# matteociccozzi/LayoutDiT

Measured on AMD Instinct MI355X. Metric: images/sec ViT-B/16 224px bs=64 fwd, higher is better.
Workload: dtype f32; 1 GPU; ViT-base/16 224x224 bs=64 f32 forward, taps [4, 6, 8, 12] (BASELINE.json configs[1]); images_per_gpu=64, global_batch=64, parallelism=dp1: batch-sharded replicas, no data-path collective, weights=synthetic seed 0, images=synthetic doc-like pages, seed 1234, rank0_placement=128 CPUs: NUMA node 0 of GPU 0000:23:00.0

## Files before the change

layoutdit_amd/csrc/api.hip:

```cpp
#include "api_internal.h"

namespace ldit {

char *err_buf()
{
    static thread_local char buf[512] = {0};
    return buf;
}

int fail(int code, const char *fmt, ...)
{
    va_list ap;
    va_start(ap, fmt);
    vsnprintf(err_buf(), 512, fmt, ap);
    va_end(ap);
    return code;
}

int ensure_dynamic_lds(const void *kern, int bytes, std::atomic<unsigned long long> &done)
{
    int dev = 0;
    LDIT_HIP_CHECK(hipGetDevice(&dev));
    const unsigned long long bit = dev >= 0 && dev < 64 ? 1ull << dev : 0ull;
    if (bit && (done.load(std::memory_order_relaxed) & bit)) return LDIT_OK;
    LDIT_HIP_CHECK(hipFuncSetAttribute(kern, hipFuncAttributeMaxDynamicSharedMemorySize, bytes));
    if (bit) done.fetch_or(bit, std::memory_order_relaxed);
    return LDIT_OK;
}

int compute_units()
{
    static std::atomic<int> cached[64];
    int dev = 0;
    if (hipGetDevice(&dev) != hipSuccess) return 256;
    const bool slot = dev >= 0 && dev < 64;
    if (slot) {
        const int c = cached[dev].load(std::memory_order_relaxed);
        if (c > 0) return c;
    }
    int n = 0;
    if (hipDeviceGetAttribute(&n, hipDeviceAttributeMultiprocessorCount, dev) != hipSuccess || n <= 0) n = 256;
    if (slot) cached[dev].store(n, std::memory_order_relaxed);
    return n;
}

namespace {
DiagSwitches read_switches()
{
    DiagSwitches d;
    auto digit = [](const char *name, int lo, int hi) {
        const char *e = getenv(name);
        return (e && e[0] >= '0' + lo && e[0] <= '0' + hi && e[1] == 0) ? e[0] - '0' : -1;
    };
    auto is = [](const char *name, char c) { const char *e = getenv(name); return e && e[0] == c; };
    d.gemm_tile = digit("LDIT_GEMM_TILE", 0, 7);
    if (const char *e = getenv("LDIT_GEMM_THIN_TILES")) d.thin_tiles = atol(e);
    d.panel_r16_vec = is("LDIT_PANEL_R16", 'v');
    d.panel_persist = is("LDIT_GEMM_PERSIST", '1');
    d.bf16_tile = digit("LDIT_GEMM_BF16_TILE", 2, 7);
    d.bf16_tile_env = getenv("LDIT_GEMM_BF16_TILE") != nullptr;
    d.bf16_tr_tile = digit("LDIT_GEMM_BF16_TR_TILE", 0, 9);
    d.bf16_tail_launch = is("LDIT_GEMM_BF16_TAIL_LAUNCH", '1');
    d.fp8_tile = digit("LDIT_GEMM_FP8_TILE", 0, 6);
    d.fp8_k16 = is("LDIT_GEMM_FP8_K16", '1');
    d.fp8_noskinny = is("LDIT_GEMM_FP8_NOSKINNY", '1');
    d.direct_epi = is("LDIT_GEMM_DIRECT_EPILOGUE", '1');
    d.attn_bf16_kt4 = is("LDIT_ATTN_BF16_KT", '4');
    d.seg_order = digit("LDIT_GEMM_SEG_ORDER", 0, 1);
    if (const char *e = getenv("LDIT_PLANES_TAIL_WAVES")) d.planes_tail_waves = atol(e);
    d.attn_bf16_nw = digit("LDIT_ATTN_BF16_NW", 4, 8);
    return d;
}
DiagSwitches &switches()
{
    static DiagSwitches d = read_switches();
    return d;
}
}

const DiagSwitches &diag() { return switches(); }
void reload_diag() { switches() = read_switches(); }

int embed(const Geo &g, const float *x, const float *pw, const float *pb, const float *cls, const float *pos, float *out,
          int batch, int img_h, int img_w, hipStream_t stream, Probe &probe)
{
    GemmArgs a{};
    a.A = x; a.W = pw; a.Y = out; a.Y2 = nullptr; a.bias = pb; a.pos = pos;
    a.M = batch * g.P; a.N = g.C; a.K = g.Kp;
    a.lda = g.in_ch * img_h * img_w;
    a.ldy = g.C;
    a.img_h = img_h; a.img_w = img_w; a.gw = g.gw; a.patches = g.P; a.patch = g.p; a.tokens = g.T;
    LDIT_RUN(probe, LDIT_K_GEMM, launch_gemm(a, EPI_EMBED, A_PATCH, stream));
    LDIT_RUN(probe, LDIT_K_OTHER, launch_cls_rows(cls, pos, out, batch, g.T, g.C, stream));
    return LDIT_OK;
}

int embed_bf16(const Geo &g, const float *x, const ImgSrc *imgs, int planes, void *patches, const void *w16, const float *pb,
               const float *cls, const float *pos, float *out, int batch, int img_h, int img_w, hipStream_t stream, Probe &probe)
{
    if (imgs)
        LDIT_RUN(probe, LDIT_K_OTHER, launch_patches_rows_images(imgs->images, imgs->half_in, imgs->heights, imgs->widths, batch, g.in_ch,
                                                                imgs->mean, imgs->std, img_h, img_w, g.p, patches, stream, planes));
    else
        LDIT_RUN(probe, LDIT_K_OTHER, launch_patches_rows(x, patches, batch, g.in_ch, img_h, img_w, g.p, stream, planes));
    GemmExtra xe = split_segments(planes);
    xe.pos = pos; xe.patches = g.P;
    LDIT_RUN(probe, LDIT_K_GEMM, launch_gemm_bf16_ex(patches, planes * g.Kp, w16, pb, out, g.C, batch * g.P, g.C, g.Kp, EPI_EMBED, nullptr,
                                                    nullptr, nullptr, xe, stream));
    LDIT_RUN(probe, LDIT_K_OTHER, launch_cls_rows(cls, pos, out, batch, g.T, g.C, stream));
    return LDIT_OK;
}

int layernorm(Build b, const float *X, const float *gamma, const float *beta, const Operand &Y, void *Yd, int64_t rows, int C, float eps, hipStream_t stream)
{
    switch (b.dtype) {
        case LDIT_F32: return launch_layernorm(X, gamma, beta, static_cast<float *>(Y.p), rows, C, eps, stream);
        case LDIT_BF16: return launch_layernorm_bf16out(X, gamma, beta, Y.p, rows, C, eps, stream);
        case LDIT_FP8: return launch_layernorm_fp8out(X, gamma, beta, Y.p, rows, C, eps, static_cast<const float *>(Y.s), stream);
        case LDIT_MXFP8:
            return b.train ? launch_layernorm_mxout_train(X, gamma, beta, Y.p, Y.s, Yd, rows, C, eps, stream)
                           : launch_layernorm_mxout(X, gamma, beta, Y.p, Y.s, rows, C, eps, stream);
        case LDIT_F32X3: case LDIT_F32X6: return launch_layernorm_splitout(X, gamma, beta, Y.p, rows, C, eps, Y.planes, stream);
        default: return fail(LDIT_EUNSUPPORTED, "layernorm: no kernel for dtype %d", b.dtype);
    }
}

int linear(Build b, const Operand &A, const void *W, const void *Ws, const float *bias, const Operand &Y, int M, int N, int K, int epi,
           const float *lam, const float *R, float *Y2, const Side &t, hipStream_t stream, float ab_scale, float out_inv_scale)
{
    switch (b.dtype) {
        case LDIT_F32: {
            GemmArgs a{};
            a.A = static_cast<const float *>(A.p); a.W = static_cast<const float *>(W); a.Y = static_cast<float *>(Y.p); a.Y2 = Y2;
            a.bias = bias; a.lam = lam; a.R = R;
            a.M = M; a.N = N; a.K = K; a.lda = A.ld; a.ldy = Y.ld;
            return launch_gemm(a, epi, A_ROWMAJOR, stream);
        }
        case LDIT_BF16: case LDIT_F32X3: case LDIT_F32X6: {
            GemmExtra x = split_segments(A.planes);
            x.Ypre = t.Ypre; x.rowscale = t.rowscale;
            if (Y.planes) { x.nsplit_out = Y.planes; epi = epi == EPI_BIAS_GELU ? EPI_GELU_SPLIT : EPI_BIAS_SPLIT; }
            return launch_gemm_bf16_ex(A.p, A.ld, W, bias, Y.p, Y.ld, M, N, K, epi, lam, R, Y2, x, stream);
        }
        case LDIT_FP8:
            return launch_gemm_fp8(A.p, A.ld, W, bias, Y.p, Y.ld, M, N, K, epi, lam, R, Y2, ab_scale, out_inv_scale,
                                   static_cast<const float *>(A.s), static_cast<const float *>(Ws), static_cast<const float *>(Y.s), stream);
        case LDIT_MXFP8:
            if (b.train && epi != EPI_BIAS)
                return launch_gemm_mxfp8_train(A.p, A.ld, A.s, W, Ws, bias, Y.p, Y.ld, Y.s, M, N, K, epi, lam, R, Y2, t.Ypre, t.rowscale, t.Yd, stream);
            return launch_gemm_mxfp8(A.p, A.ld, A.s, W, Ws, bias, Y.p, Y.ld, Y.s, M, N, K, epi, lam, R, Y2, stream);
        default: return fail(LDIT_EUNSUPPORTED, "linear: no kernel for dtype %d", b.dtype);
    }
}

int attention(Build b, const void *Q, const void *K, const void *V, int ldq, int ldk, int ldv, const Operand &O, int B, int N, int H, int D,
              float scale, hipStream_t stream, float *lse, void *Ob, void *Od, int plane_in)
{
    switch (b.dtype) {
        case LDIT_F32:
            return launch_attention(static_cast<const float *>(Q), static_cast<const float *>(K), static_cast<const float *>(V),
                                    static_cast<float *>(O.p), B, N, H, D, ldq, ldk, ldv, O.ld, scale, stream);
        case LDIT_BF16:
            return b.train ? launch_attention_bf16_lse(Q, K, V, O.p, lse, B, N, H, D, ldq, ldk, ldv, O.ld, scale, stream)
                           : launch_attention_bf16(Q, K, V, O.p, B, N, H, D, ldq, ldk, ldv, O.ld, scale, stream);
        case LDIT_FP8:
            return launch_attention_bf16_fp8out(Q, K, V, O.p, B, N, H, D, ldq, ldk, ldv, O.ld, scale, static_cast<const float *>(O.s), stream);
        case LDIT_MXFP8:
            return b.train ? launch_attention_bf16_mxout_train(Q, K, V, O.p, O.s, lse, Ob, Od, B, N, H, D, ldq, ldk, ldv, O.ld, scale, stream)
                           : launch_attention_bf16_mxout(Q, K, V, O.p, O.s, B, N, H, D, ldq, ldk, ldv, O.ld, scale, stream);
        case LDIT_F32X3: case LDIT_F32X6:
            return (O.planes == 2 ? launch_attention_planes2 : launch_attention_planes3)(Q, K, V, O.p, B, N, H, D, ldq, plane_in, O.ld, stream);
        default: return fail(LDIT_EUNSUPPORTED, "attention: no kernel for dtype %d", b.dtype);
    }
}

int run_layer(Build b, const Geo &g, int batch, float eps, const Layer &d, hipStream_t stream, Probe &probe)
{
    const int M = batch * g.T, C = g.C, F = g.F;
    const char *q = static_cast<const char *>(d.qkv.p), *k = q + d.qk_bytes, *v = k + d.qk_bytes;
    const Operand mid = operand(d.h_mid, nullptr, C), out = operand(d.h_out, nullptr, C);
    const PackedLayer &pv = *d.v, &pw = *d.w;
    LDIT_RUN(probe, LDIT_K_LAYERNORM, layernorm(b, d.h_in, d.vec(pv.ln1_w), d.vec(pv.ln1_b), d.y1, d.y1d, M, C, eps, stream));
    LDIT_RUN(probe, LDIT_K_GEMM, linear(b, d.y1, d.mat(pw.wqkv), d.W + pw.sw_qkv, d.bqkv, d.qkv, M, 3 * C, C, EPI_BIAS, nullptr, nullptr, nullptr, Side{}, stream));
    LDIT_RUN(probe, LDIT_K_ATTENTION, attention(b, q, k, v, d.qkv.ld, d.qkv.ld, d.qkv.ld, d.o, batch, g.T, g.H, g.D, d.scale, stream, d.lse, d.ob, d.od,
                                                d.qkv.planes ? d.qkv.ld / d.qkv.planes : 0));
    LDIT_RUN(probe, LDIT_K_GEMM, linear(b, d.o, d.mat(pw.wo), d.W + pw.sw_o, d.vec(pv.bo), mid, M, C, C, EPI_SCALE_RESID, d.vec(pv.lam1), d.h_in, nullptr, d.s_o, stream));
    LDIT_RUN(probe, LDIT_K_LAYERNORM, layernorm(b, d.h_mid, d.vec(pv.ln2_w), d.vec(pv.ln2_b), d.y2, d.y2d, M, C, eps, stream));
    LDIT_RUN(probe, LDIT_K_GEMM, linear(b, d.y2, d.mat(pw.w1), d.W + pw.sw_1, d.vec(pv.b1), d.hid, M, F, C, EPI_BIAS_GELU, nullptr, nullptr, nullptr, d.s_fc1, stream));
    LDIT_RUN(probe, LDIT_K_GEMM, linear(b, d.hid, d.mat(pw.w2), d.W + pw.sw_2, d.vec(pv.b2), out, M, C, F, EPI_SCALE_RESID, d.vec(pv.lam2), d.h_mid, d.tap, d.s_fc2, stream));
    return LDIT_OK;
}

namespace {

Geo embed_geo(int64_t in_ch, int64_t img_h, int64_t img_w, int64_t p, int64_t C)
{
    Geo g{};
    g.C = (int)C; g.p = (int)p; g.in_ch = (int)in_ch; g.gh = (int)(img_h / p); g.gw = (int)(img_w / p);
    g.P = g.gh * g.gw; g.T = g.P + 1; g.Kp = (int)(in_ch * p * p);
    return g;
}

int embed_bf16_entry(const char *name, const void *x, const ImgSrc *imgs, const void *patch_w_bf16, const void *patch_b, const void *cls,
                     const void *pos, void *out, void *scratch, int64_t B, int64_t in_ch, int64_t img_h, int64_t img_w, int64_t p, int64_t C,
                     ldit_stream stream)
{
    if (B <= 0 || (imgs && B > 65535) || in_ch <= 0 || img_h <= 0 || img_w <= 0 || p <= 0 || C <= 0) return fail(LDIT_EINVAL, "%s: empty problem", name);
    if (img_h % p || img_w % p)
        return fail(LDIT_EINVAL, "%s: %s %lldx%lld is not a multiple of patch %lld", name, imgs ? "target" : "image", (long long)img_h, (long long)img_w, (long long)p);
    if ((imgs ? !imgs->images || !imgs->heights || !imgs->widths : !x) || !patch_w_bf16 || !patch_b || !cls || !pos || !out || !scratch)
        return fail(LDIT_EINVAL, "%s: null operand", name);
    if (imgs && !(imgs->std > 0.0f)) return fail(LDIT_EINVAL, "%s: std must be positive", name);
    if (!aligned16(out) || !aligned16(pos) || !aligned16(scratch) || !aligned16(patch_w_bf16) || (C & 3))
        return fail(LDIT_EINVAL, "%s: out / pos / scratch / patch_w must be 16-byte aligned, C a multiple of 4", name);
    const int64_t P = (img_h / p) * (img_w / p), Kp = in_ch * p * p;
    if (Kp % 64) return fail(LDIT_EUNSUPPORTED, "%s: in_ch*p*p = %lld must be a multiple of 64", name, (long long)Kp);
    if (B * in_ch * img_h * img_w >= (1ll << 31) || B * (P + 1) * C >= (1ll << 31) || B * P * Kp >= (1ll << 31))
        return fail(LDIT_EUNSUPPORTED, "%s: operand exceeds 2^31 elements", name);
    Probe probe;
    return embed_bf16(embed_geo(in_ch, img_h, img_w, p, C), static_cast<const float *>(x), imgs, 1, scratch, patch_w_bf16,
                      static_cast<const float *>(patch_b), static_cast<const float *>(cls), static_cast<const float *>(pos), static_cast<float *>(out),
                      (int)B, (int)img_h, (int)img_w, static_cast<hipStream_t>(stream), probe);
}
// ... 516 lines not shown
```

layoutdit_amd/csrc/attention_f32.hip:

```cpp
#include "ldit_common.h"

#ifdef LDIT_GEMM_STAMPS
__device__ unsigned long long *g_attn32_stamps = nullptr;
#define A32_STAMP(var) const unsigned long long var = __builtin_amdgcn_s_memtime()
#else
#define A32_STAMP(var)
#endif

namespace ldit {

namespace {

constexpr int KSTR = 68;
constexpr int VSTR = 64;

template <int KT, int NW>
__global__ void __launch_bounds__(NW * 64, NW == 4 ? 2 : NW / 4) attention_f32(const float *__restrict__ Q, const float *__restrict__ K,
                                                     const float *__restrict__ V, float *__restrict__ O, int N, int H,
                                                     int ldq, int ldk, int ldv, int ldo, float scale, int nqg)
{
    constexpr int KROWS = KT * 32;
    extern __shared__ __attribute__((aligned(16))) char smem[];
    float *Ks = reinterpret_cast<float *>(smem);
    float *Vs = Ks + KROWS * KSTR;

    const int tid = threadIdx.x, lane = tid & 63;
    const int wave = __builtin_amdgcn_readfirstlane(tid >> 6);
    const int li = lane & 31, lh = lane >> 5;
    const int bid = blockIdx.x;
    const int qg = bid % nqg, bh = bid / nqg, head = bh % H, b = bh / H;
    const int qt = qg * NW + wave;
    const bool active = qt * 32 < N;
    const size_t tok0 = (size_t)b * N;
#ifdef LDIT_GEMM_STAMPS
    unsigned long long ph[4] = {0, 0, 0, 0};
#endif
    A32_STAMP(t_begin);

    float q[32];
    {
        int qrow = qt * 32 + li;
        qrow = qrow < N ? qrow : N - 1;
        const f32x4 *qp = reinterpret_cast<const f32x4 *>(Q + (tok0 + qrow) * ldq + head * 64 + 32 * lh);
#pragma unroll
        for (int u = 0; u < 8; ++u) {
            const f32x4 t = qp[u];
            q[4 * u + 0] = t[0]; q[4 * u + 1] = t[1]; q[4 * u + 2] = t[2]; q[4 * u + 3] = t[3];
        }
    }

    f32x16 o[2];
#pragma unroll
    for (int e = 0; e < 16; ++e) { o[0][e] = 0.0f; o[1][e] = 0.0f; }
    float m_run = -INFINITY, l_run = 0.0f;

    for (int c0 = 0; c0 < N; c0 += KROWS) {
        const int nkeys = (N - c0) < KROWS ? (N - c0) : KROWS;
        const int ktiles = (nkeys + 31) >> 5;
        A32_STAMP(t0);
        if (c0) __syncthreads();
        {
            constexpr int PER = (32 * 16) / (NW * 64) > 0 ? (32 * 16) / (NW * 64) : 1;
            static_assert((32 * 16) % (NW * 64) == 0, "a key tile must split evenly over the threads");
            constexpr int BATCH = 4;
#pragma unroll
            for (int e = 0; e < PER; ++e)
#pragma unroll
                for (int k0 = 0; k0 < KT; k0 += BATCH) {
                    f32x4 kv[BATCH], vv[BATCH];
#pragma unroll
                    for (int i = 0; i < BATCH; ++i) {
                        const int kt = k0 + i, u = kt * 512 + e * NW * 64 + tid, row = u >> 4, c4 = (u & 15) * 4;
                        kv[i] = f32x4{0.f, 0.f, 0.f, 0.f};
                        vv[i] = f32x4{0.f, 0.f, 0.f, 0.f};
                        if (kt < KT && kt < ktiles && row < nkeys) {
                            kv[i] = *reinterpret_cast<const f32x4 *>(K + (tok0 + c0 + row) * ldk + head * 64 + c4);
                            vv[i] = *reinterpret_cast<const f32x4 *>(V + (tok0 + c0 + row) * ldv + head * 64 + c4);
                        }
                    }
#pragma unroll
                    for (int i = 0; i < BATCH; ++i) {
                        const int kt = k0 + i, u = kt * 512 + e * NW * 64 + tid, row = u >> 4, c4 = (u & 15) * 4;
                        if (kt < KT && kt < ktiles) {
                            *reinterpret_cast<f32x4 *>(Ks + row * KSTR + c4) = kv[i];
                            *reinterpret_cast<f32x4 *>(Vs + row * VSTR + c4) = vv[i];
                        }
                    }
                }
        }
        __syncthreads();
        if (!active) continue;
        A32_STAMP(t1);

        f32x16 s[KT];
#pragma unroll
        for (int kt = 0; kt < KT; ++kt) {
#pragma unroll
            for (int e = 0; e < 16; ++e) s[kt][e] = 0.0f;
            if (kt < ktiles) {
                const float *kr = Ks + (kt * 32 + li) * KSTR + 32 * lh;
#pragma unroll
                for (int u = 0; u < 8; ++u) {
                    const f32x4 kf = *reinterpret_cast<const f32x4 *>(kr + 4 * u);
#pragma unroll
                    for (int e = 0; e < 4; ++e)
                        s[kt] = __builtin_amdgcn_mfma_f32_32x32x2f32(kf[e], q[4 * u + e], s[kt], 0, 0, 0);
                }
            }
        }
#ifdef LDIT_GEMM_STAMPS
        asm volatile("s_nop 0" ::"v"(s[0][0]), "v"(s[KT - 1][0]));
#endif
        A32_STAMP(t2);
        float mx = -INFINITY;
#pragma unroll
        for (int kt = 0; kt < KT; ++kt) {
            if (kt < ktiles) {
                const bool partial = (kt + 1) * 32 > nkeys;
#pragma unroll
                for (int r = 0; r < 16; ++r) {
                    float v = s[kt][r] * scale;
                    if (partial && (kt * 32 + 8 * (r >> 2) + 4 * lh + (r & 3)) >= nkeys) v = -INFINITY;
                    s[kt][r] = v;
                    mx = fmaxf(mx, v);
                }
            }
        }
        mx = fmaxf(mx, __shfl_xor(mx, 32, 64));
        const float m_new = fmaxf(m_run, mx);
        const float alpha = __expf(m_run - m_new);
        m_run = m_new;
        float lsum = 0.0f;
#pragma unroll
        for (int kt = 0; kt < KT; ++kt) {
            if (kt < ktiles) {
#pragma unroll
                for (int r = 0; r < 16; ++r) {
                    const float pv = __expf(s[kt][r] - m_new);
                    s[kt][r] = pv;
                    lsum += pv;
                }
            }
        }
        l_run = l_run * alpha + lsum;
        if (c0) {
#pragma unroll
            for (int e = 0; e < 16; ++e) { o[0][e] *= alpha; o[1][e] *= alpha; }
        }
        A32_STAMP(t3);
#pragma unroll
        for (int kt = 0; kt < KT; ++kt) {
            if (kt < ktiles) {
                const int left = nkeys - kt * 32;
#pragma unroll
                for (int r = 0; r < 16; ++r) {
                    if (8 * (r >> 2) + (r & 3) >= left) continue;
                    const float *vr = Vs + (kt * 32 + 8 * (r >> 2) + 4 * lh + (r & 3)) * VSTR + li;
                    o[0] = __builtin_amdgcn_mfma_f32_32x32x2f32(vr[0], s[kt][r], o[0], 0, 0, 0);
                    o[1] = __builtin_amdgcn_mfma_f32_32x32x2f32(vr[32], s[kt][r], o[1], 0, 0, 0);
                }
            }
        }
#ifdef LDIT_GEMM_STAMPS
        asm volatile("s_nop 0" ::"v"(o[0][0]), "v"(o[1][0]));
        ph[0] += t1 - t0 + (c0 ? 0 : t0 - t_begin); ph[1] += t2 - t1; ph[2] += t3 - t2; ph[3] += __builtin_amdgcn_s_memtime() - t3;
#endif
    }

    if (!active) return;
#ifdef LDIT_GEMM_STAMPS
    if (g_attn32_stamps && wave == 0 && lane == 0) {
        unsigned long long *d = g_attn32_stamps + (size_t)blockIdx.x * 6;
        d[0] = ph[0]; d[1] = ph[1]; d[2] = ph[2]; d[3] = ph[3]; d[5] = __builtin_amdgcn_s_memtime() - t_begin;
    }
#endif
    const float l = l_run + __shfl_xor(l_run, 32, 64);
    const float inv = 1.0f / l;
    const int qrow = qt * 32 + li;
    if (qrow < N) {
        float *op = O + (tok0 + qrow) * ldo + head * 64 + 4 * lh;
#pragma unroll
        for (int dt = 0; dt < 2; ++dt)
#pragma unroll
            for (int g = 0; g < 4; ++g) {
                f32x4 t = {o[dt][4 * g + 0] * inv, o[dt][4 * g + 1] * inv, o[dt][4 * g + 2] * inv, o[dt][4 * g + 3] * inv};
                *reinterpret_cast<f32x4 *>(op + dt * 32 + 8 * g) = t;
            }
    }
}

}

int launch_attention(const float *Q, const float *K, const float *V, float *O, int B, int N, int H, int D, int ldq,
                     int ldk, int ldv, int ldo, float scale, hipStream_t stream)
{
    if (B <= 0 || N <= 0 || H <= 0) return fail(LDIT_EINVAL, "attention: empty problem");
    if (D != 64) return fail(LDIT_EUNSUPPORTED, "attention: head_dim=%d, only 64 is implemented", D);
    if (!Q || !K || !V || !O) return fail(LDIT_EINVAL, "attention: null operand");
    if ((ldq | ldk | ldv | ldo) & 3) return fail(LDIT_EINVAL, "attention: row strides must be multiples of 4 floats");
    if (!aligned16(Q) || !aligned16(K) || !aligned16(V) || !aligned16(O)) return fail(LDIT_EINVAL, "attention: operands must be 16-byte aligned");
    constexpr int KT = 7;
    constexpr int lds = KT * 32 * (KSTR + VSTR) * 4;
    const int nqt = (N + 31) / 32;
    auto go = [&](auto kern, int nw, std::atomic<unsigned long long> &attr_done) -> int {
        if (int rc = ensure_dynamic_lds(reinterpret_cast<const void *>(kern), lds, attr_done)) return rc;
        const int nqg = (nqt + nw - 1) / nw;
        hipLaunchKernelGGL(kern, dim3((unsigned)(B * H * nqg)), dim3(nw * 64), lds, stream, Q, K, V, O, N, H, ldq, ldk, ldv, ldo,
                           scale, nqg);
        LDIT_HIP_CHECK(hipGetLastError());
        return LDIT_OK;
    };
    static std::atomic<unsigned long long> set8{0}, set4{0};
    const long wgs8 = (long)B * H * ((nqt + 7) / 8);
    if (wgs8 <= 128 && nqt > 4) { if (int rc = go(attention_f32<KT, 4>, 4, set4)) return rc; }
    else if (int rc = go(attention_f32<KT, 8>, 8, set8)) return rc;
    LDIT_HIP_CHECK(hipGetLastError());
    return LDIT_OK;
}

}

#ifdef LDIT_GEMM_STAMPS
extern "C" int ldit_dbg_set_attn32_stamps(void *buf)
{
    unsigned long long *p = static_cast<unsigned long long *>(buf);
    return hipMemcpyToSymbol(HIP_SYMBOL(g_attn32_stamps), &p, sizeof(p)) == hipSuccess ? 0 : -3;
}
#endif
```

layoutdit_amd/csrc/ldit_common.h:

```cpp
#pragma once
#include <hip/hip_runtime.h>

#include <atomic>
#include <cstdarg>
#include <cstdint>
#include <cstdio>

#include "ldit.h"

namespace ldit {

typedef float f32x2 __attribute__((ext_vector_type(2)));
typedef float f32x4 __attribute__((ext_vector_type(4)));
typedef float f32x16 __attribute__((ext_vector_type(16)));

char *err_buf();
int fail(int code, const char *fmt, ...);

#define LDIT_HIP_CHECK(expr)                                                                              \
    do {                                                                                                  \
        hipError_t e__ = (expr);                                                                          \
        if (e__ != hipSuccess) return ::ldit::fail(LDIT_EHIP, "%s: %s", #expr, hipGetErrorString(e__));   \
    } while (0)

static inline bool aligned16(const void *p) { return (reinterpret_cast<uintptr_t>(p) & 15u) == 0; }

int ensure_dynamic_lds(const void *kern, int bytes, std::atomic<unsigned long long> &done);
#define LDIT_DYN_LDS(kern, bytes)                                                                               \
    do {                                                                                                        \
        static std::atomic<unsigned long long> done__{0};                                                       \
        if (int rc__ = ::ldit::ensure_dynamic_lds(reinterpret_cast<const void *>(kern), (bytes), done__)) return rc__; \
    } while (0)

int compute_units();

struct DiagSwitches {
    int gemm_tile = -1;
    long thin_tiles = 192;
    bool panel_r16_vec = false;
    bool panel_persist = false;
    int bf16_tile = -1;
    bool bf16_tile_env = false;
    int bf16_tr_tile = -1;
    bool bf16_tail_launch = false;
    int fp8_tile = -1;
    bool fp8_k16 = false, fp8_noskinny = false;
    bool direct_epi = false;
    bool attn_bf16_kt4 = false;
    int attn_bf16_nw = -1;
    long planes_tail_waves = 700;
    int seg_order = -1;
};
const DiagSwitches &diag();
void reload_diag();

__device__ __forceinline__ float erf_fast(float a)
{
    const float t = fabsf(a), s = a * a;
    float r = fmaf(-1.72853470e-5f, t, 3.83197126e-4f);
    const float u = fmaf(-3.88396438e-3f, t, 2.42546219e-2f);
    r = fmaf(r, s, u);
    r = fmaf(r, t, -1.06777877e-1f);
    r = fmaf(r, t, -6.34846687e-1f);
    r = fmaf(r, t, -1.28717512e-1f);
    r = fmaf(r, t, -t);
    const float big = copysignf(1.0f - __expf(r), a);
    float q = -5.96761703e-4f;
    q = fmaf(q, s, 4.99119423e-3f);
    q = fmaf(q, s, -2.67681349e-2f);
    q = fmaf(q, s, 1.12819925e-1f);
    q = fmaf(q, s, -3.76125336e-1f);
    q = fmaf(q, s, 1.28379166e-1f);
    const float small = fmaf(q, a, a);
    return t > 0.927734375f ? big : small;
}

__device__ __forceinline__ float gelu_erf(float v) { return 0.5f * v * (1.0f + erf_fast(v * 0.70710678118654752440f)); }

__device__ __forceinline__ float gelu_lp(float v)
{
    const float w = v * __builtin_fmaf(v * v, -0.10294324f, -2.30220819f);
    return v * __builtin_amdgcn_rcpf(1.0f + __builtin_amdgcn_exp2f(w));
}

__device__ __forceinline__ void gelu_and_grad_lp(float v, float &gelu, float &grad)
{
    const float v2 = v * v;
    const float w = v * __builtin_fmaf(v2, -0.10294324f, -2.30220819f);
    const float s = __builtin_amdgcn_rcpf(1.0f + __builtin_amdgcn_exp2f(w));
    const float vs = v * s;
    gelu = vs;
    grad = __builtin_fmaf(vs - vs * s, __builtin_fmaf(v2, 0.21406445f, 1.59576912f), s);
}

__device__ __forceinline__ unsigned pack_fp8x4(float a, float b, float c, float d)
{
    const float lim = 448.0f;
    a = fminf(fmaxf(a, -lim), lim); b = fminf(fmaxf(b, -lim), lim);
    c = fminf(fmaxf(c, -lim), lim); d = fminf(fmaxf(d, -lim), lim);
    int w = 0;
    w = __builtin_amdgcn_cvt_pk_fp8_f32(a, b, w, false);
    w = __builtin_amdgcn_cvt_pk_fp8_f32(c, d, w, true);
    return (unsigned)w;
}

__device__ __forceinline__ unsigned umax32(unsigned a, unsigned b) { return a > b ? a : b; }

__device__ __forceinline__ unsigned mx_scale_byte(unsigned amax)
{
    if (amax >= 0x7f800000u) return 0xFFu;
    if (amax == 0u) return 0u;
    int e = (int)(amax >> 23) - 135 + ((amax & 0x7fffffu) > 0x600000u ? 1 : 0);
    e = e < -127 ? -127 : (e > 127 ? 127 : e);
    return (unsigned)(e + 127);
}

__device__ __forceinline__ float mx_inv_scale(unsigned b) { return b >= 254u ? 1.0f : __uint_as_float((254u - b) << 23); }

__device__ __forceinline__ float mx_scale_value(unsigned b)
{
    return b == 0u ? __uint_as_float(0x00400000u) : (b == 255u ? __uint_as_float(0x7fc00000u) : __uint_as_float(b << 23));
}

typedef __bf16 mx_bf16x4 __attribute__((ext_vector_type(4)));

__device__ __forceinline__ mx_bf16x4 mx_dequant_bf16x4(unsigned pk, unsigned b)
{
    const float s = mx_scale_value(b);
    return mx_bf16x4{(__bf16)(__builtin_amdgcn_cvt_f32_fp8((int)pk, 0) * s), (__bf16)(__builtin_amdgcn_cvt_f32_fp8((int)pk, 1) * s),
                     (__bf16)(__builtin_amdgcn_cvt_f32_fp8((int)pk, 2) * s), (__bf16)(__builtin_amdgcn_cvt_f32_fp8((int)pk, 3) * s)};
}

enum AMode { A_ROWMAJOR = 0, A_PATCH = 1,
             A_CONV3 = 2 };
enum Epi { EPI_BIAS = 0, EPI_BIAS_GELU = 1, EPI_SCALE_RESID = 2, EPI_EMBED = 3,
           EPI_F32 = 4,
           EPI_GELU_BWD = 5,
           EPI_GELU_SPLIT = 6,
           EPI_BIAS_SPLIT = 7 };

struct GemmExtra {
    void *Ypre = nullptr;
    const float *rowscale = nullptr;
    const void *aux = nullptr;
    int ldaux = 0;
    int splits = 1;
    const void *zeros = nullptr;
    const float *pos = nullptr;
    int patches = 0;
    int nseg = 0;
    unsigned seg_a = 0, seg_w = 0;
    int seg_inner = 0;
    int nsplit_out = 0;
    float *colsum = nullptr;
    int tail_rows = 0;
};

template <int S>
__device__ __forceinline__ void split_bf16_planes(float x, __bf16 (&p)[S])
{
#pragma unroll
    for (int s = 0; s < S; ++s) {
        p[s] = (__bf16)x;
        x -= (float)p[s];
    }
}

struct GemmArgs {
    const float *A;
    const float *W;
    float *Y;
    float *Y2;
    const float *bias;
    const float *lam;
    const float *R;
    const float *pos;
    int M, N, K;
    int lda, ldy;
    int img_h, img_w, gw, patches, patch, tokens;
    int conv_h, conv_w, conv_c;
    const float *zeros;
#ifdef LDIT_GEMM_STAMPS
    unsigned long long *stamps;
#endif
};

int launch_gemm(const GemmArgs &a, int epi, int amode, hipStream_t stream);
int launch_gemm_panel(const GemmArgs &a, int epi, int amode, hipStream_t stream, int height = 304);
int launch_gemm_thin(const GemmArgs &a, int epi, hipStream_t stream);
bool gemm_thin_prefers(int M, int N);

int launch_layernorm(const float *X, const float *g, const float *b, float *Y, int64_t rows, int C, float eps,
                     hipStream_t stream);
int launch_layernorm_bf16out(const float *X, const float *g, const float *b, void *Y, int64_t rows, int C, float eps,
                             hipStream_t stream);
int launch_attention_bf16(const void *Q, const void *K, const void *V, void *O, int B, int N, int H, int D, int ldq, int ldk,
                          int ldv, int ldo, float scale, hipStream_t stream);
int launch_attention(const float *Q, const float *K, const float *V, float *O, int B, int N, int H, int D, int ldq,
                     int ldk, int ldv, int ldo, float scale, hipStream_t stream);
int launch_cls_rows(const float *cls, const float *pos, float *out, int B, int tokens, int C, hipStream_t stream);
int launch_tap_to_map(const float *tap, float *out, int B, int Gh, int Gw, int C, float scale, hipStream_t stream);
int launch_tap_to_map_bwd(const float *dmap, float *dtap, int B, int Gh, int Gw, int C, float scale, hipStream_t stream);
// ... 105 lines not shown
```

layoutdit_amd/ops.py:

```python
from __future__ import annotations

import ctypes as C
from typing import Optional, Sequence

import torch

from . import _lib


def _device(*tensors) -> torch.device:
    dev = None
    for t in tensors:
        if t is None:
            continue
        if dev is None:
            dev = t.device
        elif t.device != dev:
            raise ValueError(f"tensor arguments live on different devices ({dev} and {t.device})")
    if dev is None or dev.type != "cuda":
        raise ValueError("expected tensors on the GPU (libldit_hip has no CPU path)")
    return dev


def _launch(dev: torch.device, fn, *args) -> None:
    with torch.cuda.device(dev):
        _lib.check(fn(*args, torch.cuda.current_stream(dev).cuda_stream))


def _req(t: torch.Tensor, name: str) -> torch.Tensor:
    if not isinstance(t, torch.Tensor) or not t.is_cuda:
        raise ValueError(f"{name}: expected a tensor on the GPU (libldit_hip has no CPU path)")
    if t.dtype != torch.float32:
        raise ValueError(f"{name}: expected float32, got {t.dtype}")
    if not t.is_contiguous():
        raise ValueError(f"{name}: expected a contiguous tensor")
    return t


def _ptr(t: Optional[torch.Tensor]):
    return None if t is None else t.data_ptr()


def linear(x: torch.Tensor, weight: torch.Tensor, bias: Optional[torch.Tensor] = None, epilogue: int = _lib.EPI_BIAS,
           lam: Optional[torch.Tensor] = None, residual: Optional[torch.Tensor] = None,
           out: Optional[torch.Tensor] = None, out2: Optional[torch.Tensor] = None) -> torch.Tensor:
    lib = _lib.load()
    x, weight = _req(x, "x"), _req(weight, "weight")
    M, K = x.shape
    N = weight.shape[0]
    if weight.shape[1] != K:
        raise ValueError(f"weight {tuple(weight.shape)} does not match x {tuple(x.shape)}")
    if out is None:
        out = torch.empty((M, N), device=x.device, dtype=torch.float32)
    for t, n in ((bias, "bias"), (lam, "lam"), (residual, "residual"), (out, "out"), (out2, "out2")):
        if t is not None:
            _req(t, n)
    _launch(_device(x, weight, bias, lam, residual, out, out2), lib.ldit_linear_f32, _ptr(x), K, _ptr(weight), _ptr(bias), _ptr(out), N, M, N, K, epilogue, _ptr(lam),
                                   _ptr(residual), _ptr(out2))
    return out


def layernorm(x: torch.Tensor, gamma: torch.Tensor, beta: torch.Tensor, eps: float = 1e-12) -> torch.Tensor:
    lib = _lib.load()
    x, gamma, beta = _req(x, "x"), _req(gamma, "gamma"), _req(beta, "beta")
    C = x.shape[-1]
    rows = x.numel() // C
    y = torch.empty_like(x)
    _launch(_device(x, gamma, beta), lib.ldit_layernorm_f32, _ptr(x), _ptr(gamma), _ptr(beta), _ptr(y), rows, C, eps)
    return y


def attention(q: torch.Tensor, k: torch.Tensor, v: torch.Tensor, heads: int, scale: Optional[float] = None) -> torch.Tensor:
    lib = _lib.load()
    for t, n in ((q, "q"), (k, "k"), (v, "v")):
        if not t.is_cuda or t.dtype != torch.float32 or t.stride(-1) != 1 or t.stride(0) != t.shape[1] * t.stride(1):
            raise ValueError(f"{n}: expected GPU float32 [B,N,H*D] with unit last stride and dense batch stride")
    B, N, HD = q.shape
    D = HD // heads
    o = torch.empty((B, N, HD), device=q.device, dtype=torch.float32)
    _launch(_device(q, k, v), lib.ldit_attention_f32, _ptr(q), _ptr(k), _ptr(v), _ptr(o), B, N, heads, D, q.stride(1), k.stride(1),
                                      v.stride(1), HD, float(D ** -0.5 if scale is None else scale))
    return o


def embed(x: torch.Tensor, patch_w: torch.Tensor, patch_b: torch.Tensor, cls: torch.Tensor, pos: torch.Tensor,
          patch: int) -> torch.Tensor:
    lib = _lib.load()
    x, patch_w, patch_b = _req(x, "x"), _req(patch_w, "patch_w"), _req(patch_b, "patch_b")
    cls, pos = _req(cls, "cls"), _req(pos, "pos")
    B, in_ch, H, W = x.shape
    Cc = patch_w.shape[0]
    T = (H // patch) * (W // patch) + 1
    out = torch.empty((B, T, Cc), device=x.device, dtype=torch.float32)
    _launch(_device(x, patch_w, patch_b, cls, pos), lib.ldit_embed_f32, _ptr(x), _ptr(patch_w), _ptr(patch_b), _ptr(cls), _ptr(pos), _ptr(out), B, in_ch, H, W,
                                  patch, Cc)
    return out


def embed_bf16(x: torch.Tensor, patch_w_bf16: torch.Tensor, patch_b: torch.Tensor, cls: torch.Tensor, pos: torch.Tensor,
               patch: int) -> torch.Tensor:
    lib = _lib.load()
    x, patch_b, cls, pos = _req(x, "x"), _req(patch_b, "patch_b"), _req(cls, "cls"), _req(pos, "pos")
    if patch_w_bf16.dtype != torch.bfloat16 or not patch_w_bf16.is_contiguous():
        raise ValueError("patch_w_bf16 must be a contiguous bfloat16 tensor")
    B, in_ch, H, W = x.shape
    Cc = patch_w_bf16.shape[0]
    P = (H // patch) * (W // patch)
    out = torch.empty((B, P + 1, Cc), device=x.device, dtype=torch.float32)
    scratch = torch.empty((B * P, in_ch * patch * patch), device=x.device, dtype=torch.bfloat16)
    _launch(_device(x, patch_w_bf16, patch_b, cls, pos), lib.ldit_embed_bf16, _ptr(x), _ptr(patch_w_bf16), _ptr(patch_b), _ptr(cls),
            _ptr(pos), _ptr(out), _ptr(scratch), B, in_ch, H, W, patch, Cc)
    return out


def tap_to_map(tap: torch.Tensor, gh: int, gw: int, scale: float) -> torch.Tensor:
    lib = _lib.load()
    tap = _req(tap, "tap")
    B, T, Cc = tap.shape
    if T != gh * gw + 1:
        raise ValueError(f"tap has {T} tokens, grid {gh}x{gw} needs {gh * gw + 1}")
    out = torch.empty((B, Cc, int(gh * scale), int(gw * scale)), device=tap.device, dtype=torch.float32)
    _launch(_device(tap), lib.ldit_tap_to_map_f32, _ptr(tap), _ptr(out), B, gh, gw, Cc, float(scale))
    return out


def _req16(t: torch.Tensor, name: str) -> torch.Tensor:
    if not isinstance(t, torch.Tensor) or not t.is_cuda or t.dtype != torch.float16 or not t.is_contiguous():
        raise ValueError(f"{name}: expected a contiguous float16 tensor on the GPU")
    return t


def widen_f16(x: torch.Tensor) -> torch.Tensor:
    lib = _lib.load()
    x = _req16(x, "x")
    out = torch.empty(x.shape, device=x.device, dtype=torch.float32)
    _launch(_device(x), lib.ldit_cast_f16_f32, _ptr(x), _ptr(out), x.numel())
    return out


def narrow_f16(x: torch.Tensor) -> torch.Tensor:
    lib = _lib.load()
    x = _req(x, "x")
    out = torch.empty(x.shape, device=x.device, dtype=torch.float16)
    _launch(_device(x), lib.ldit_cast_f32_f16, _ptr(x), _ptr(out), x.numel())
    return out


class _TapToMapFn(torch.autograd.Function):

    @staticmethod
    def forward(ctx, tap, gh, gw, scale):
        ctx.geom = (gh, gw, float(scale))
        return tap_to_map(tap.detach(), gh, gw, scale)

    @staticmethod
    def backward(ctx, dmap):
        gh, gw, scale = ctx.geom
        lib = _lib.load()
        dmap = _req(dmap.contiguous(), "dmap")
        B, Cc = dmap.shape[0], dmap.shape[1]
        dtap = torch.empty((B, gh * gw + 1, Cc), device=dmap.device, dtype=torch.float32)
        _launch(_device(dmap), lib.ldit_tap_to_map_bwd_f32, _ptr(dmap), _ptr(dtap), B, gh, gw, Cc, scale)
        return dtap, None, None, None


def tap_to_map_autograd(tap: torch.Tensor, gh: int, gw: int, scale: float) -> torch.Tensor:
    return _TapToMapFn.apply(tap, gh, gw, scale)


def preprocess(images: Sequence[torch.Tensor], size=224, mean: float = 0.5, std: float = 0.5) -> torch.Tensor:
    lib = _lib.load()
    imgs, ptrs, hs, ws, half, ch = image_list_args(images)
    B = len(imgs)
    out_h, out_w = (size, size) if isinstance(size, int) else (int(size[0]), int(size[1]))
    out = torch.empty((B, ch, out_h, out_w), device=imgs[0].device, dtype=torch.float32)
    if half:
        _launch(_device(*imgs), lib.ldit_preprocess_f16, ptrs, hs, ws, B, ch, mean, std, out_h, out_w, _ptr(out))
    else:
        _launch(_device(*imgs), lib.ldit_preprocess_f32, ptrs, hs, ws, B, ch, mean, std, out_h, out_w, _ptr(out))
    return out


def image_list_args(images: Sequence[torch.Tensor]):
    if len(images) == 0:
        raise ValueError("empty image list")
    half = images[0].dtype == torch.float16
    imgs = [(_req16 if half else _req)(t, f"images[{i}]") for i, t in enumerate(images)]
    ch = imgs[0].shape[0]
    if any(t.dim() != 3 or t.shape[0] != ch for t in imgs):
        raise ValueError("every image must be [C, h, w] with the same C")
    B = len(imgs)
    ptrs = (C.c_void_p * B)(*[t.data_ptr() for t in imgs])
    hs = (C.c_int32 * B)(*[t.shape[1] for t in imgs])
    ws = (C.c_int32 * B)(*[t.shape[2] for t in imgs])
    return imgs, ptrs, hs, ws, half, ch


def embed_bf16_images(images: Sequence[torch.Tensor], patch_w_bf16: torch.Tensor, patch_b: torch.Tensor, cls: torch.Tensor,
                      pos: torch.Tensor, patch: int, size=224, mean: float = 0.5, std: float = 0.5) -> torch.Tensor:
    lib = _lib.load()
    imgs, ptrs, hs, ws, half, ch = image_list_args(images)
    patch_b, cls, pos = _req(patch_b, "patch_b"), _req(cls, "cls"), _req(pos, "pos")
    if patch_w_bf16.dtype != torch.bfloat16 or not patch_w_bf16.is_contiguous():
        raise ValueError("patch_w_bf16 must be a contiguous bfloat16 tensor")
    out_h, out_w = (size, size) if isinstance(size, int) else (int(size[0]), int(size[1]))
    B, Cc = len(imgs), patch_w_bf16.shape[0]
    P = (out_h // patch) * (out_w // patch)
    dev = imgs[0].device
    out = torch.empty((B, P + 1, Cc), device=dev, dtype=torch.float32)
    scratch = torch.empty((B * P, ch * patch * patch), device=dev, dtype=torch.bfloat16)
    _launch(_device(*imgs, patch_w_bf16, patch_b, cls, pos), lib.ldit_embed_bf16_images, ptrs, hs, ws, int(half), mean, std,
            _ptr(patch_w_bf16), _ptr(patch_b), _ptr(cls), _ptr(pos), _ptr(out), _ptr(scratch), B, ch, out_h, out_w, patch, Cc)
    return out


def cast_bf16(x: torch.Tensor) -> torch.Tensor:
    lib = _lib.load()
    x = _req(x, "x")
    out = torch.empty(x.shape, device=x.device, dtype=torch.bfloat16)
    _launch(_device(x), lib.ldit_cast_f32_bf16, _ptr(x), _ptr(out), x.numel())
    return out


def linear_bf16(x: torch.Tensor, weight: torch.Tensor, bias: Optional[torch.Tensor] = None, epilogue: int = _lib.EPI_BIAS,
                lam: Optional[torch.Tensor] = None, residual: Optional[torch.Tensor] = None,
                out: Optional[torch.Tensor] = None, out2: Optional[torch.Tensor] = None) -> torch.Tensor:
    lib = _lib.load()
    for t, n in ((x, "x"), (weight, "weight")):
        if not t.is_cuda or t.dtype != torch.bfloat16 or not t.is_contiguous():
            raise ValueError(f"{n}: expected a contiguous bfloat16 GPU tensor")
    M, K = x.shape
    N = weight.shape[0]
# ... 839 lines not shown
```

Before: 3414 images/sec.

## Add persistent pipelined f32 attention kernel with direct-to-LDS K/V prefetch

Adds a persistent attention kernel, used when the whole key sequence fits in one LDS tile. Each block loops over (batch, head) pairs and prefetches the next head's K and Q with global_load_lds while the current head's PV product runs. It computes softmax in a single pass, since every key is resident, and XOR-swizzles the K rows in LDS instead of padding them. The old online-softmax kernel stays as the fallback, and the shared pieces are factored into helper functions. In exchange, the new path relies on inline assembly that manipulates m0, needs hand-placed waitcnt and barriers, and leaves one of the eight waves idle when the sequence has 197 tokens.

```diff
diff --git a/layoutdit_amd/csrc/api.hip b/layoutdit_amd/csrc/api.hip
--- a/layoutdit_amd/csrc/api.hip
+++ b/layoutdit_amd/csrc/api.hip
@@ -69,6 +69,7 @@
     d.seg_order = digit("LDIT_GEMM_SEG_ORDER", 0, 1);
     if (const char *e = getenv("LDIT_PLANES_TAIL_WAVES")) d.planes_tail_waves = atol(e);
     d.attn_bf16_nw = digit("LDIT_ATTN_BF16_NW", 4, 8);
+    d.attn_f32_pipe = digit("LDIT_ATTN_F32_PIPE", 0, 1);
     return d;
 }
 DiagSwitches &switches()
diff --git a/layoutdit_amd/csrc/attention_f32.hip b/layoutdit_amd/csrc/attention_f32.hip
--- a/layoutdit_amd/csrc/attention_f32.hip
+++ b/layoutdit_amd/csrc/attention_f32.hip
@@ -13,6 +13,107 @@
 
 constexpr int KSTR = 68;
 constexpr int VSTR = 64;
+
+
+__device__ __forceinline__ void attn_load_q(float (&q)[32], const float *qrow_ptr)
+{
+    const f32x4 *qp = reinterpret_cast<const f32x4 *>(qrow_ptr);
+#pragma unroll
+    for (int u = 0; u < 8; ++u) {
+        const f32x4 t = qp[u];
+        q[4 * u + 0] = t[0]; q[4 * u + 1] = t[1]; q[4 * u + 2] = t[2]; q[4 * u + 3] = t[3];
+    }
+}
+
+template <int KT, bool SWZ>
+__device__ __forceinline__ void attn_scores(f32x16 (&s)[KT], const float *Ks, const float (&q)[32], int ktiles, int li, int lh)
+{
+#pragma unroll
+    for (int kt = 0; kt < KT; ++kt) {
+#pragma unroll
+        for (int e = 0; e < 16; ++e) s[kt][e] = 0.0f;
+        if (kt < ktiles) {
+            const float *kr = SWZ ? Ks + (kt * 32 + li) * 64 : Ks + (kt * 32 + li) * KSTR + 32 * lh;
+#pragma unroll
+            for (int u = 0; u < 8; ++u) {
+                const f32x4 kf = *reinterpret_cast<const f32x4 *>(SWZ ? kr + 4 * ((8 * lh + u) ^ (li & 15)) : kr + 4 * u);
+#pragma unroll
+                for (int e = 0; e < 4; ++e)
+                    s[kt] = __builtin_amdgcn_mfma_f32_32x32x2f32(kf[e], q[4 * u + e], s[kt], 0, 0, 0);
+            }
+        }
+    }
+}
+
+template <int KT>
+__device__ __forceinline__ float attn_softmax(f32x16 (&s)[KT], int nkeys, int ktiles, float scale, int lh, float &m_run, float &l_run)
+{
+    float mx = -INFINITY;
+#pragma unroll
+    for (int kt = 0; kt < KT; ++kt) {
+        if (kt < ktiles) {
+            const bool partial = (kt + 1) * 32 > nkeys;
+#pragma unroll
+            for (int r = 0; r < 16; ++r) {
+                float v = s[kt][r] * scale;
+                if (partial && (kt * 32 + 8 * (r >> 2) + 4 * lh + (r & 3)) >= nkeys) v = -INFINITY;
+                s[kt][r] = v;
+                mx = fmaxf(mx, v);
+            }
+        }
+    }
+    mx = fmaxf(mx, __shfl_xor(mx, 32, 64));
+    const float m_new = fmaxf(m_run, mx);
+    const float alpha = __expf(m_run - m_new);
+    m_run = m_new;
+    float lsum = 0.0f;
+#pragma unroll
+    for (int kt = 0; kt < KT; ++kt) {
+        if (kt < ktiles) {
+#pragma unroll
+            for (int r = 0; r < 16; ++r) {
+                const float pv = __expf(s[kt][r] - m_new);
+                s[kt][r] = pv;
+                lsum += pv;
+            }
+        }
+    }
+    l_run = l_run * alpha + lsum;
+    return alpha;
+}
+
+template <int KT>
+__device__ __forceinline__ void attn_pv(f32x16 (&o)[2], const f32x16 (&s)[KT], const float *Vs, int nkeys, int ktiles, int li, int lh)
+{
+#pragma unroll
+    for (int kt = 0; kt < KT; ++kt) {
+        if (kt < ktiles) {
+            const int left = nkeys - kt * 32;
+#pragma unroll
+            for (int r = 0; r < 16; ++r) {
+                if (8 * (r >> 2) + (r & 3) >= left) continue;
+                const float *vr = Vs + (kt * 32 + 8 * (r >> 2) + 4 * lh + (r & 3)) * VSTR + li;
+                o[0] = __builtin_amdgcn_mfma_f32_32x32x2f32(vr[0], s[kt][r], o[0], 0, 0, 0);
+                o[1] = __builtin_amdgcn_mfma_f32_32x32x2f32(vr[32], s[kt][r], o[1], 0, 0, 0);
+            }
+        }
+    }
+}
+
+__device__ __forceinline__ void attn_store(const f32x16 (&o)[2], float l_run, float *op)
+{
+    const float l = l_run + __shfl_xor(l_run, 32, 64);
+    const float inv = 1.0f / l;
+    if (op) {
+#pragma unroll
+        for (int dt = 0; dt < 2; ++dt)
+#pragma unroll
+            for (int g = 0; g < 4; ++g) {
+                f32x4 t = {o[dt][4 * g + 0] * inv, o[dt][4 * g + 1] * inv, o[dt][4 * g + 2] * inv, o[dt][4 * g + 3] * inv};
+                *reinterpret_cast<f32x4 *>(op + dt * 32 + 8 * g) = t;
+            }
+    }
+}
 
 template <int KT, int NW>
 __global__ void __launch_bounds__(NW * 64, NW == 4 ? 2 : NW / 4) attention_f32(const float *__restrict__ Q, const float *__restrict__ K,
@@ -41,12 +142,7 @@
     {
         int qrow = qt * 32 + li;
         qrow = qrow < N ? qrow : N - 1;
-        const f32x4 *qp = reinterpret_cast<const f32x4 *>(Q + (tok0 + qrow) * ldq + head * 64 + 32 * lh);
-#pragma unroll
-        for (int u = 0; u < 8; ++u) {
-            const f32x4 t = qp[u];
-            q[4 * u + 0] = t[0]; q[4 * u + 1] = t[1]; q[4 * u + 2] = t[2]; q[4 * u + 3] = t[3];
-        }
+        attn_load_q(q, Q + (tok0 + qrow) * ldq + head * 64 + 32 * lh);
     }
 
     f32x16 o[2];
@@ -93,74 +189,18 @@
         A32_STAMP(t1);
 
         f32x16 s[KT];
-#pragma unroll
-        for (int kt = 0; kt < KT; ++kt) {
-#pragma unroll
-            for (int e = 0; e < 16; ++e) s[kt][e] = 0.0f;
-            if (kt < ktiles) {
-                const float *kr = Ks + (kt * 32 + li) * KSTR + 32 * lh;
-#pragma unroll
-                for (int u = 0; u < 8; ++u) {
-                    const f32x4 kf = *reinterpret_cast<const f32x4 *>(kr + 4 * u);
-#pragma unroll
-                    for (int e = 0; e < 4; ++e)
-                        s[kt] = __builtin_amdgcn_mfma_f32_32x32x2f32(kf[e], q[4 * u + e], s[kt], 0, 0, 0);
-                }
-            }
-        }
+        attn_scores<KT, false>(s, Ks, q, ktiles, li, lh);
 #ifdef LDIT_GEMM_STAMPS
         asm volatile("s_nop 0" ::"v"(s[0][0]), "v"(s[KT - 1][0]));
 #endif
         A32_STAMP(t2);
-        float mx = -INFINITY;
-#pragma unroll
-        for (int kt = 0; kt < KT; ++kt) {
-            if (kt < ktiles) {
-                const bool partial = (kt + 1) * 32 > nkeys;
-#pragma unroll
-                for (int r = 0; r < 16; ++r) {
-                    float v = s[kt][r] * scale;
-                    if (partial && (kt * 32 + 8 * (r >> 2) + 4 * lh + (r & 3)) >= nkeys) v = -INFINITY;
-                    s[kt][r] = v;
-                    mx = fmaxf(mx, v);
-                }
-            }
-        }
-        mx = fmaxf(mx, __shfl_xor(mx, 32, 64));
-        const float m_new = fmaxf(m_run, mx);
-        const float alpha = __expf(m_run - m_new);
-        m_run = m_new;
-        float lsum = 0.0f;
-#pragma unroll
-        for (int kt = 0; kt < KT; ++kt) {
-            if (kt < ktiles) {
-#pragma unroll
-                for (int r = 0; r < 16; ++r) {
-                    const float pv = __expf(s[kt][r] - m_new);
-                    s[kt][r] = pv;
-                    lsum += pv;
-                }
-            }
-        }
-        l_run = l_run * alpha + lsum;
+        const float alpha = attn_softmax<KT>(s, nkeys, ktiles, scale, lh, m_run, l_run);
         if (c0) {
 #pragma unroll
             for (int e = 0; e < 16; ++e) { o[0][e] *= alpha; o[1][e] *= alpha; }
         }
         A32_STAMP(t3);
-#pragma unroll
-        for (int kt = 0; kt < KT; ++kt) {
-            if (kt < ktiles) {
-                const int left = nkeys - kt * 32;
-#pragma unroll
-                for (int r = 0; r < 16; ++r) {
-                    if (8 * (r >> 2) + (r & 3) >= left) continue;
-                    const float *vr = Vs + (kt * 32 + 8 * (r >> 2) + 4 * lh + (r & 3)) * VSTR + li;
-                    o[0] = __builtin_amdgcn_mfma_f32_32x32x2f32(vr[0], s[kt][r], o[0], 0, 0, 0);
-                    o[1] = __builtin_amdgcn_mfma_f32_32x32x2f32(vr[32], s[kt][r], o[1], 0, 0, 0);
-                }
-            }
-        }
+        attn_pv<KT>(o, s, Vs, nkeys, ktiles, li, lh);
 #ifdef LDIT_GEMM_STAMPS
         asm volatile("s_nop 0" ::"v"(o[0][0]), "v"(o[1][0]));
         ph[0] += t1 - t0 + (c0 ? 0 : t0 - t_begin); ph[1] += t2 - t1; ph[2] += t3 - t2; ph[3] += __builtin_amdgcn_s_memtime() - t3;
@@ -174,20 +214,134 @@
         d[0] = ph[0]; d[1] = ph[1]; d[2] = ph[2]; d[3] = ph[3]; d[5] = __builtin_amdgcn_s_memtime() - t_begin;
     }
 #endif
-    const float l = l_run + __shfl_xor(l_run, 32, 64);
-    const float inv = 1.0f / l;
     const int qrow = qt * 32 + li;
-    if (qrow < N) {
-        float *op = O + (tok0 + qrow) * ldo + head * 64 + 4 * lh;
-#pragma unroll
-        for (int dt = 0; dt < 2; ++dt)
-#pragma unroll
-            for (int g = 0; g < 4; ++g) {
-                f32x4 t = {o[dt][4 * g + 0] * inv, o[dt][4 * g + 1] * inv, o[dt][4 * g + 2] * inv, o[dt][4 * g + 3] * inv};
-                *reinterpret_cast<f32x4 *>(op + dt * 32 + 8 * g) = t;
-            }
-    }
-}
+    attn_store(o, l_run, qrow < N ? O + (tok0 + qrow) * ldo + head * 64 + 4 * lh : nullptr);
+}
+
+__device__ __forceinline__ void glds16_sbase(const void *ubase, unsigned voff_bytes, unsigned lds_dst)
+{
+    unsigned keep;
+    asm volatile("s_nop 4\n\ts_mov_b32 %0, m0\n\ts_mov_b32 m0, %3\n\ts_nop 0\n\tglobal_load_lds_dwordx4 %1, %2\n\ts_mov_b32 m0, %0"
+                 : "=&s"(keep)
+                 : "v"(voff_bytes), "s"(ubase), "s"(lds_dst)
+                 : "memory");
+}
+
+template <int KT>
+__global__ void __launch_bounds__(512, 2) attention_f32_pipe(const float *__restrict__ Q, const float *__restrict__ K,
+                                                             const float *__restrict__ V, float *__restrict__ O, int N, int H,
+                                                             int ldq, int ldk, int ldv, int ldo, float scale, int nheads)
+{
+    constexpr int KROWS = KT * 32;
+    extern __shared__ __attribute__((aligned(16))) char smem[];
+    float *Ks = reinterpret_cast<float *>(smem);
+    float *Vs = Ks + KROWS * 64;
+
+    const int tid = threadIdx.x, lane = tid & 63;
+    const int wave = __builtin_amdgcn_readfirstlane(tid >> 6);
+    const int li = lane & 31, lh = lane >> 5;
+    const int qt = wave;
+    const bool active = qt * 32 < N;
+    const int step = (int)gridDim.x;
+
+    const int prow = 4 * wave + (lane >> 4), pch = lane & 15;
+    const int dtiles = (N + 31) >> 5;
+    const int lastrow = N - 1 - 32 * (dtiles - 1);
+    const int crow = prow < lastrow ? prow : lastrow;
+    const unsigned kch = 16u * (unsigned)(pch ^ (prow & 15)), vch = 16u * (unsigned)pch;
+    const unsigned koff = 4u * (unsigned)prow * (unsigned)ldk + kch, koff_last = 4u * (unsigned)crow * (unsigned)ldk + kch;
+    const unsigned voff = 4u * (unsigned)prow * (unsigned)ldv + vch, voff_last = 4u * (unsigned)crow * (unsigned)ldv + vch;
+    const unsigned lds0 = __builtin_amdgcn_readfirstlane((unsigned)(uintptr_t)((__attribute__((address_space(3))) char *)smem));
+    const unsigned kdst = lds0 + 1024u * (unsigned)wave, vdst = kdst + (unsigned)(KROWS * 256);
+    auto issue = [&](const float *head_base, int ld, unsigned off, unsigned off_last, unsigned dst) {
+#pragma unroll
+        for (int u = 0; u < KT; ++u)
+            if (u < dtiles) glds16_sbase(head_base + (size_t)(32 * u) * ld, u == dtiles - 1 ? off_last : off, dst + 8192u * u);
+    };
+    auto q_row = [&](int bh) {
+        int qrow = qt * 32 + li;
+        qrow = qrow < N ? qrow : N - 1;
+        return Q + ((size_t)(bh / H) * N + qrow) * ldq + (bh % H) * 64 + 32 * lh;
+    };
+
+    int bh = blockIdx.x;
+    A32_STAMP(t_head);
+#ifdef LDIT_GEMM_STAMPS
+    unsigned long long t_mark = t_head;
+    int slot = 0;
+#endif
+    float q[32];
+    issue(K + (size_t)(bh / H) * N * ldk + (bh % H) * 64, ldk, koff, koff_last, kdst);
+    if (active) attn_load_q(q, q_row(bh));
+    asm volatile("s_waitcnt vmcnt(0)" ::: "memory");
+
+    for (; bh < nheads; bh += step) {
+        const int head = bh % H, b = bh / H;
+        const size_t tok0 = (size_t)b * N;
+        int nkeys = N;
+        asm volatile("" : "+s"(nkeys));
+        const int ktiles = (nkeys + 31) >> 5;
+        __builtin_amdgcn_s_barrier();
+        asm volatile("" ::: "memory");
+        issue(V + tok0 * ldv + head * 64, ldv, voff, voff_last, vdst);
+        A32_STAMP(t1);
+
+        f32x16 s[KT];
+        float m_run = -INFINITY, l_run = 0.0f;
+        if (active) {
+            attn_scores<KT, true>(s, Ks, q, ktiles, li, lh);
+#ifdef LDIT_GEMM_STAMPS
+            asm volatile("s_nop 0" ::"v"(s[0][0]), "v"(s[KT - 1][0]));
+#endif
+        }
+        A32_STAMP(t2);
+        if (active) {
+            attn_softmax<KT>(s, nkeys, ktiles, scale, lh, m_run, l_run);
+#ifdef LDIT_GEMM_STAMPS
+            asm volatile("s_nop 0" ::"v"(s[0][0]), "v"(s[KT - 1][0]));
+#endif
+        }
+        A32_STAMP(t3);
+        asm volatile("s_waitcnt vmcnt(0)" ::: "memory");
+        __builtin_amdgcn_s_barrier();
+        asm volatile("" ::: "memory");
+        const int nxt = bh + step;
+        if (nxt < nheads) {
+            issue(K + (size_t)(nxt / H) * N * ldk + (nxt % H) * 64, ldk, koff, koff_last, kdst);
+            if (active) attn_load_q(q, q_row(nxt));
+        }
+        A32_STAMP(t4);
+        f32x16 o[2];
+        if (active) {
+#pragma unroll
+            for (int e = 0; e < 16; ++e) { o[0][e] = 0.0f; o[1][e] = 0.0f; }
+            attn_pv<KT>(o, s, Vs, nkeys, ktiles, li, lh);
+#ifdef LDIT_GEMM_STAMPS
+            asm volatile("s_nop 0" ::"v"(o[0][0]), "v"(o[1][0]));
+#endif
+        }
+        A32_STAMP(t5);
+        asm volatile("s_waitcnt vmcnt(0)" ::: "memory");
+        if (active) {
+            const int qrow = qt * 32 + li;
+            attn_store(o, l_run, qrow < N ? O + (tok0 + qrow) * ldo + head * 64 + 4 * lh : nullptr);
+        }
+#ifdef LDIT_GEMM_STAMPS
+        {
+            const unsigned long long t6 = __builtin_amdgcn_s_memtime();
+            if (g_attn32_stamps && wave == 0 && lane == 0 && slot < 4) {
+                unsigned long long *d = g_attn32_stamps + ((size_t)blockIdx.x * 4 + slot) * 8;
+                d[0] = t1 - t_mark; d[1] = t2 - t1; d[2] = t3 - t2; d[3] = t4 - t3; d[4] = t5 - t4; d[5] = t6 - t5; d[6] = t6 - t_mark;
+                d[7] = (unsigned long long)bh + 1;
+            }
+            t_mark = t6;
+            ++slot;
+        }
+#endif
+    }
+}
+
+std::atomic<long long> g_pipe_launches{0};
 
 }
 
@@ -202,6 +356,18 @@
     constexpr int KT = 7;
     constexpr int lds = KT * 32 * (KSTR + VSTR) * 4;
     const int nqt = (N + 31) / 32;
+    const long heads = (long)B * H;
+    const int cus = compute_units(), mode = diag().attn_f32_pipe;
+    if (N <= KT * 32 && mode != 0 && (mode == 1 || heads >= 2L * cus) && heads < (1L << 31) && ldk < (1 << 23) && ldv < (1 << 23)) {
+        constexpr int lds_pipe = KT * 32 * (64 + VSTR) * 4;
+        LDIT_DYN_LDS((attention_f32_pipe<KT>), lds_pipe);
+        const unsigned grid = (unsigned)(heads < cus ? heads : cus);
+        hipLaunchKernelGGL((attention_f32_pipe<KT>), dim3(grid), dim3(512), lds_pipe, stream, Q, K, V, O, N, H, ldq, ldk, ldv, ldo, scale,
+                           (int)heads);
+        LDIT_HIP_CHECK(hipGetLastError());
+        g_pipe_launches.fetch_add(1, std::memory_order_relaxed);
+        return LDIT_OK;
+    }
     auto go = [&](auto kern, int nw, std::atomic<unsigned long long> &attr_done) -> int {
         if (int rc = ensure_dynamic_lds(reinterpret_cast<const void *>(kern), lds, attr_done)) return rc;
         const int nqg = (nqt + nw - 1) / nw;
@@ -220,6 +386,8 @@
 
 }
 
+extern "C" long long ldit_dbg_attn32_pipe_launches(void) { return ldit::g_pipe_launches.load(std::memory_order_relaxed); }
+
 #ifdef LDIT_GEMM_STAMPS
 extern "C" int ldit_dbg_set_attn32_stamps(void *buf)
 {
diff --git a/layoutdit_amd/csrc/ldit_common.h b/layoutdit_amd/csrc/ldit_common.h
--- a/layoutdit_amd/csrc/ldit_common.h
+++ b/layoutdit_amd/csrc/ldit_common.h
@@ -48,6 +48,7 @@
     bool direct_epi = false;
     bool attn_bf16_kt4 = false;
     int attn_bf16_nw = -1;
+    int attn_f32_pipe = -1;
     long planes_tail_waves = 700;
     int seg_order = -1;
 };
diff --git a/layoutdit_amd/ops.py b/layoutdit_amd/ops.py
--- a/layoutdit_amd/ops.py
+++ b/layoutdit_amd/ops.py
@@ -70,14 +70,20 @@
     return y
 
 
-def attention(q: torch.Tensor, k: torch.Tensor, v: torch.Tensor, heads: int, scale: Optional[float] = None) -> torch.Tensor:
+def attention(q: torch.Tensor, k: torch.Tensor, v: torch.Tensor, heads: int, scale: Optional[float] = None,
+              out: Optional[torch.Tensor] = None) -> torch.Tensor:
     lib = _lib.load()
     for t, n in ((q, "q"), (k, "k"), (v, "v")):
         if not t.is_cuda or t.dtype != torch.float32 or t.stride(-1) != 1 or t.stride(0) != t.shape[1] * t.stride(1):
             raise ValueError(f"{n}: expected GPU float32 [B,N,H*D] with unit last stride and dense batch stride")
     B, N, HD = q.shape
     D = HD // heads
-    o = torch.empty((B, N, HD), device=q.device, dtype=torch.float32)
+    if out is None:
+        o = torch.empty((B, N, HD), device=q.device, dtype=torch.float32)
+    else:
+        o = out
+        if not o.is_cuda or o.dtype != torch.float32 or not o.is_contiguous() or tuple(o.shape) != (B, N, HD) or o.device != q.device:
+            raise ValueError("out: expected a contiguous GPU float32 [B,N,H*D] tensor on the operands' device")
     _launch(_device(q, k, v), lib.ldit_attention_f32, _ptr(q), _ptr(k), _ptr(v), _ptr(o), B, N, heads, D, q.stride(1), k.stride(1),
                                       v.stride(1), HD, float(D ** -0.5 if scale is None else scale))
     return o
```

Result: no change. 3433 images/sec, median of 6 (+0.6%).
